# traveller59/spconv

Hardware: NVIDIA H100
Metric: active-voxels/sec fwd+bwd SubMConv3d 3^3 C=64 (higher is better)
Workload: dtype fp16

## Files before the change

spconv_b200/csrc/gemm_tc.cu:

```cuda
#include "gemm.cuh"
#include "wgmma.cuh"
#include <cuda.h>
#include <atomic>
#include <mutex>
#include <stdlib.h>

namespace spx {

constexpr int TC_TILE_M = 128;
constexpr int TC_CONS_WARPS = 8;
constexpr int TC_PROD_WARPS = 2;
constexpr int TC_PROD_THREADS = TC_PROD_WARPS * 32;
constexpr int TC_TMA_WARP = TC_CONS_WARPS + TC_PROD_WARPS;
constexpr int TC_SCHED_WARP = TC_TMA_WARP + 1;
constexpr int TC_THREADS = 3 * 128;
constexpr int TC_INFO_DEPTH = 4;
constexpr int TC_INFO_READERS = TC_PROD_WARPS + TC_CONS_WARPS + 1;
constexpr int TC_MAX_STAGES = 8;
constexpr int TC_SMEM_BUDGET = 200 * 1024;

struct TcParams {
    const uint8_t *x;
    int xb;
    int span_b, b_subtiles, b_sub_bytes, b_bytes, b_mn_major, b_kstep16_mn;
    int b_transposed;
    const float *w;
    int c_in, c_out;
    int w_inner_elems;
    int span_b_elems;
    int n;
    int ab_bf16;
    int stages, a_stage_bytes, stage_bytes, idx_bytes;
    int64_t rows;
    const int32_t *tile_table;
    const int32_t *sched_rec;
    int *sched_state;
    const int32_t *argsort;
    int kv, words, reverse;
    void *y;
    int out_dtype;
    int epi_mode;
    const void *bias;
    int act; float alpha;
    const float *scale, *bias_f32;
    const int8_t *output_add;
    float output_add_scale;
    const float *in_scale, *add_scale, *out_scale;
};

struct BitIter {
    uint32_t m0, m1, m2, m3;
    __device__ __forceinline__ BitIter(const uint32_t (&t)[4]) : m0(t[0]), m1(t[1]), m2(t[2]), m3(t[3]) {}
    __device__ __forceinline__ int next() {
        if (m0) { int b = __ffs(m0) - 1; m0 &= m0 - 1; return b; }
        if (m1) { int b = __ffs(m1) - 1; m1 &= m1 - 1; return 32 + b; }
        if (m2) { int b = __ffs(m2) - 1; m2 &= m2 - 1; return 64 + b; }
        if (m3) { int b = __ffs(m3) - 1; m3 &= m3 - 1; return 96 + b; }
        return -1;
    }
};

template <int OUT>
__device__ __forceinline__ void store2(uint8_t *dst, float a, float b) {
    if constexpr (OUT == SPX_F32) {
        *reinterpret_cast<float2 *>(dst) = make_float2(a, b);
    } else if constexpr (OUT == SPX_F16) {
        *reinterpret_cast<__half2 *>(dst) = __floats2half2_rn(a, b);
    } else if constexpr (OUT == SPX_BF16) {
        *reinterpret_cast<__nv_bfloat162 *>(dst) = __floats2bfloat162_rn(a, b);
    } else {
        const int qa = (int)fminf(fmaxf(rintf(a), -128.f), 127.f), qb = (int)fminf(fmaxf(rintf(b), -128.f), 127.f);
        *reinterpret_cast<uint16_t *>(dst) = (uint16_t)((uint32_t)(uint8_t)(int8_t)qa | ((uint32_t)(uint8_t)(int8_t)qb << 8));
    }
}

template <int OUT> struct OutElem { static constexpr int bytes = OUT == SPX_F32 ? 4 : (OUT == SPX_I8 ? 1 : 2); };

template <int OUT>
__device__ __forceinline__ float load_bias(const void *bias, int j) {
    if constexpr (OUT == SPX_F32) return ((const float *)bias)[j];
    else if constexpr (OUT == SPX_F16) return __half2float(((const __half *)bias)[j]);
    else return __bfloat162float(((const __nv_bfloat16 *)bias)[j]);
}

template <int OUT, bool INT8_MODE, int N, typename Acc, bool PLAIN = false>
__device__ __forceinline__ void epilogue_frag(const TcParams &p, const float *ec, const Acc (&acc)[N / 2], int64_t dst_lo,
                                              int64_t dst_hi, int lane) {
    if constexpr (!INT8_MODE && !PLAIN) {
        if (p.bias == nullptr && p.act == SPX_ACT_NONE) {
            epilogue_frag<OUT, false, N, Acc, true>(p, ec, acc, dst_lo, dst_hi, lane);
            return;
        }
    }
    constexpr int EB = OutElem<OUT>::bytes;
    const bool has_bias = !PLAIN && (INT8_MODE ? (p.bias_f32 != nullptr) : (p.bias != nullptr));
#pragma unroll
    for (int h = 0; h < 2; ++h) {
        const int64_t dst = h ? dst_hi : dst_lo;
        if (dst < 0) continue;
        uint8_t *row_ptr = (uint8_t *)p.y + dst * (int64_t)N * EB;
#pragma unroll
        for (int nb = 0; nb < N / 8; ++nb) {
            const int col = nb * 8 + 2 * (lane & 3);
            float f[2];
#pragma unroll
            for (int j = 0; j < 2; ++j) {
                const Acc v = acc[nb * 4 + 2 * h + j];
                if constexpr (!INT8_MODE) {
                    f[j] = (float)v;
                    if (has_bias) f[j] += ec[col + j];
                } else {
                    f[j] = (float)(int32_t)v * ec[col + j];
                    if (has_bias) f[j] += ec[N + col + j];
                    if (p.output_add) f[j] += (float)p.output_add[dst * (int64_t)N + col + j] * p.output_add_scale;
                }
                if (!PLAIN && p.act != SPX_ACT_NONE) f[j] = apply_act(f[j], p.act, p.alpha);
            }
            store2<OUT>(row_ptr + col * EB, f[0], f[1]);
        }
    }
}

template <int OUT, int N>
__device__ __forceinline__ void epilogue_fp8(const TcParams &p, const float *ec, const float (&acc)[N / 2],
                                             int64_t dst_lo, int64_t dst_hi, int lane, float add_s, float out_s) {
    constexpr int EB = OUT == SPX_F32 ? 4 : (OUT == SPX_E4M3 ? 1 : 2);
    const float *bias = p.bias_f32 ? ec + N : nullptr;
    const void *add = (const void *)p.output_add;
#pragma unroll
    for (int h = 0; h < 2; ++h) {
        const int64_t dst = h ? dst_hi : dst_lo;
        if (dst < 0) continue;
        uint8_t *row_ptr = (uint8_t *)p.y + dst * (int64_t)N * EB;
#pragma unroll
        for (int nb = 0; nb < N / 8; ++nb) {
            const int col = nb * 8 + 2 * (lane & 3);
            float f[2];
#pragma unroll
            for (int j = 0; j < 2; ++j) {
                const float a = add ? load_out_elem<OUT>(add, dst * (int64_t)N + col + j) : 0.f;
                f[j] = fp8_epilogue(acc[nb * 4 + 2 * h + j], ec[col + j], bias, col + j, add != nullptr, a, add_s,
                                    p.act, p.alpha);
            }
            if constexpr (OUT == SPX_E4M3)
                *reinterpret_cast<uint16_t *>(row_ptr + col) = float2_to_e4m3x2(__fdiv_rn(f[0], out_s), __fdiv_rn(f[1], out_s));
            else
                store2<OUT>(row_ptr + col * EB, f[0], f[1]);
        }
    }
}

template <int KIND, int N, typename Acc>
__device__ __forceinline__ void mma_step(Acc (&acc)[N / 2], uint64_t a, uint64_t b, int b_mn, int bf16) {
    if constexpr (KIND == KIND_F16) {
        if (bf16) {
            if (b_mn) Wgmma<N>::template bf16<0, 1>(acc, a, b, 1u);
            else Wgmma<N>::template bf16<0, 0>(acc, a, b, 1u);
        } else {
            if (b_mn) Wgmma<N>::template f16<0, 1>(acc, a, b, 1u);
            else Wgmma<N>::template f16<0, 0>(acc, a, b, 1u);
        }
    } else if constexpr (KIND == KIND_TF32) {
        Wgmma<N>::tf32(acc, a, b, 1u);
    } else if constexpr (KIND == KIND_I8) {
        Wgmma<N>::s8(acc, a, b, 1u);
    } else {
        Wgmma<N>::e4m3(acc, a, b, 1u);
    }
}

template <int KIND, int CPR, int N>
__device__ __forceinline__ void tc_gather_gemm_body(const CUtensorMap &tmap_w, const TcParams &p) {
    using Acc = typename std::conditional<KIND == KIND_I8, int32_t, float>::type;
    constexpr int LG_CPR = CPR == 2 ? 1 : CPR == 4 ? 2 : CPR == 8 ? 3 : CPR == 16 ? 4 : 5;
    constexpr int RPI = 32 / CPR;
    constexpr int XB = CPR * 16;
    constexpr int SPAN_A = XB < 128 ? XB : 128;
    constexpr int LG_SPAN_A = SPAN_A == 128 ? 7 : (SPAN_A == 64 ? 6 : 5);
    constexpr int A_SUB_BYTES = TC_TILE_M * SPAN_A;
    constexpr int A_SUBTILES = XB / SPAN_A;
    constexpr int Q_A = SPAN_A / 32;
    constexpr int ROWS_PW = TC_TILE_M / TC_PROD_WARPS;
    constexpr int ITERS = ROWS_PW / RPI > 0 ? ROWS_PW / RPI : 1;
    static_assert(ROWS_PW * CPR >= 32, "a producer warp must cover at least one full cp.async instruction");

    extern __shared__ __align__(1024) uint8_t smem_raw[];
    const uint32_t raw_addr = smem_u32(smem_raw);
    const uint32_t pad = (1024u - (raw_addr & 1023u)) & 1023u;
    uint8_t *smem = smem_raw + pad;
    const uint32_t smem_base = raw_addr + pad;

    const uint32_t idx_off = (uint32_t)p.stages * p.stage_bytes;
    uint64_t *bars = reinterpret_cast<uint64_t *>(smem + idx_off + 2u * p.idx_bytes);
    uint64_t *full = bars;
    uint64_t *empty = bars + TC_MAX_STAGES;
    uint64_t *idx_full = bars + 2 * TC_MAX_STAGES;
    uint64_t *idx_empty = bars + 2 * TC_MAX_STAGES + 2;
    uint64_t *info_full = bars + 2 * TC_MAX_STAGES + 4;
    uint64_t *info_empty = bars + 2 * TC_MAX_STAGES + 4 + TC_INFO_DEPTH;
    int32_t *info = reinterpret_cast<int32_t *>(bars + 2 * TC_MAX_STAGES + 4 + 2 * TC_INFO_DEPTH);
    float *ec = reinterpret_cast<float *>(smem + idx_off + 2u * p.idx_bytes + 1024u);

    const int warp = threadIdx.x >> 5;
    const int lane = threadIdx.x & 31;
    const int64_t num_tiles = (p.rows + TC_TILE_M - 1) / TC_TILE_M;

    auto read_info = [&](int n, uint32_t (&tm)[4]) -> int {
        const int e = n & (TC_INFO_DEPTH - 1);
        mbar_wait_silent(&info_full[e], (uint32_t)((n / TC_INFO_DEPTH) & 1));
        const volatile int32_t *r = info + e * 8;
        const int tile = r[0];
        tm[0] = (uint32_t)r[1]; tm[1] = (uint32_t)r[2]; tm[2] = (uint32_t)r[3]; tm[3] = (uint32_t)r[4];
        __syncwarp();
        if (lane == 0) mbar_arrive(&info_empty[e]);
        return tile;
    };

    if (threadIdx.x == 0) {
        for (int s = 0; s < p.stages; ++s) {
            mbar_init(&full[s], TC_PROD_THREADS + 1);
            mbar_init(&empty[s], TC_CONS_WARPS);
        }
        for (int a = 0; a < 2; ++a) {
            mbar_init(&idx_full[a], 1);
            mbar_init(&idx_empty[a], TC_PROD_WARPS + TC_CONS_WARPS);
        }
        for (int e = 0; e < TC_INFO_DEPTH; ++e) {
            mbar_init(&info_full[e], 1);
            mbar_init(&info_empty[e], TC_INFO_READERS);
        }
        mbar_fence_init();
        tma_prefetch_desc(&tmap_w);
    }
    for (int j = threadIdx.x; j < N; j += TC_THREADS) {
        if constexpr (KIND == KIND_I8) {
            ec[j] = __ldg(p.scale + j);
            if (p.bias_f32) ec[N + j] = __ldg(p.bias_f32 + j);
        } else if constexpr (KIND == KIND_E4M3) {
            ec[j] = __fmul_rn(__ldg(p.in_scale), __ldg(p.scale + j));
            if (p.bias_f32) ec[N + j] = __ldg(p.bias_f32 + j);
        } else if (p.bias) {
            if constexpr (KIND == KIND_TF32) ec[j] = load_bias<SPX_F32>(p.bias, j);
            else ec[j] = p.out_dtype == SPX_F16 ? load_bias<SPX_F16>(p.bias, j) : load_bias<SPX_BF16>(p.bias, j);
        }
    }
    __syncthreads();

    if (warp >= TC_CONS_WARPS && warp < TC_TMA_WARP) {
        const int pw = warp - TC_CONS_WARPS;
        const int r0 = lane >> LG_CPR;
        const uint32_t byte_in_row = (uint32_t)(lane & (CPR - 1)) << 4;
        const uint8_t *x_lane = p.x + byte_in_row;
        uint32_t dst_off[ITERS];
#pragma unroll
        for (int itc = 0; itc < ITERS; ++itc) {
            const uint32_t row_in_tile = (uint32_t)(pw * ROWS_PW + r0 + itc * RPI);
            const uint32_t sub = byte_in_row >> LG_SPAN_A;
            const uint32_t within = byte_in_row & (uint32_t)(SPAN_A - 1);
            dst_off[itc] = sub * (uint32_t)A_SUB_BYTES + swizzle_offset((row_in_tile << LG_SPAN_A) + within, SPAN_A);
        }
        int stage = 0; uint32_t phase = 0;
        for (int n = 0;; ++n) {
            uint32_t tm[4];
            if (read_info(n, tm) < 0) break;
            const int buf = n & 1;
            mbar_wait_silent(&idx_full[buf], (uint32_t)((n >> 1) & 1));
            const int32_t *idx_lane = reinterpret_cast<const int32_t *>(smem + idx_off + (size_t)buf * p.idx_bytes) +
                                      pw * ROWS_PW + r0;
            BitIter it(tm);
            int k = it.next();
            int32_t ridx[ITERS];
            if (k >= 0) {
#pragma unroll
                for (int itc = 0; itc < ITERS; ++itc) ridx[itc] = idx_lane[k * 128 + itc * RPI];
            }
            while (k >= 0) {
                mbar_wait_silent(&empty[stage], phase ^ 1u);
                const uint32_t a_stage = smem_base + (uint32_t)stage * p.stage_bytes;
#pragma unroll
                for (int itc = 0; itc < ITERS; ++itc)
                    cp_async_16(a_stage + dst_off[itc], x_lane + (int64_t)max(ridx[itc], 0) * XB,
                                ridx[itc] >= 0 ? 16u : 0u);
                cp_async_mbar_arrive_noinc(&full[stage]);
                k = it.next();
                if (k >= 0) {
#pragma unroll
                    for (int itc = 0; itc < ITERS; ++itc) ridx[itc] = idx_lane[k * 128 + itc * RPI];
                }
                if (++stage == p.stages) { stage = 0; phase ^= 1u; }
            }
            __syncwarp();
            if (lane == 0) mbar_arrive(&idx_empty[buf]);
        }
    } else if (warp == TC_TMA_WARP) {
        int stage = 0; uint32_t phase = 0;
        for (int n = 0;; ++n) {
            uint32_t tm[4];
            if (read_info(n, tm) < 0) break;
            BitIter it(tm);
            for (int k = it.next(); k >= 0; k = it.next()) {
                mbar_wait_silent(&empty[stage], phase ^ 1u);
                const int kw = p.reverse ? p.kv - 1 - k : k;
                const uint32_t b_stage = smem_base + (uint32_t)stage * p.stage_bytes + p.a_stage_bytes;
                if (p.b_transposed) {
                    const int i4s = p.c_in >> 2;
                    const float *wk = p.w + (int64_t)kw * p.c_in;
                    for (int q = lane; q < p.c_out * i4s; q += 32) {
                        const int o = q / i4s, i4 = (q - o * i4s) * 4;
                        const float4 v = __ldg(reinterpret_cast<const float4 *>(wk + (int64_t)o * p.kv * p.c_in + i4));
                        const uint32_t kb = (uint32_t)o * 4u;
                        const uint32_t sub = kb / (uint32_t)p.span_b, within = kb % (uint32_t)p.span_b;
                        const float vv[4] = {v.x, v.y, v.z, v.w};
#pragma unroll
                        for (int t = 0; t < 4; ++t) {
                            const uint32_t off = sub * (uint32_t)p.b_sub_bytes +
                                                 swizzle_offset((uint32_t)(i4 + t) * (uint32_t)p.span_b + within, (uint32_t)p.span_b);
                            asm volatile("st.shared.f32 [%0], %1;" ::"r"(b_stage + off), "f"(vv[t]) : "memory");
                        }
                    }
                    fence_proxy_async_smem();
                    __syncwarp();
                    if (lane == 0) mbar_arrive(&full[stage]);
                } else if (lane == 0) {
                    mbar_arrive_expect_tx(&full[stage], (uint32_t)p.b_bytes);
                    for (int sb = 0; sb < p.b_subtiles; ++sb)
                        tma_load_2d(b_stage + sb * p.b_sub_bytes, &tmap_w, &full[stage],
                                    kw * p.w_inner_elems + sb * p.span_b_elems, 0);
                }
                __syncwarp();
                if (++stage == p.stages) { stage = 0; phase ^= 1u; }
            }
        }
    } else if (warp == TC_SCHED_WARP) {
        const uint32_t blk_bytes = (uint32_t)(p.kv + 1) * 512u;
        for (int n = 0;; ++n) {
            const int b = n & 1, e = n & (TC_INFO_DEPTH - 1);
            mbar_wait_silent(&idx_empty[b], (uint32_t)(((n >> 1) & 1) ^ 1));
            mbar_wait_silent(&info_empty[e], (uint32_t)(((n / TC_INFO_DEPTH) & 1) ^ 1));
            int tile = -1;
            if (lane == 0) {
                const int ticket = atomicAdd(p.sched_state, 1);
                int4 r0 = make_int4(-1, 1, 0, 0), r1 = make_int4(0, 0, 0, 0);
                if ((int64_t)ticket < num_tiles) {
                    const int4 *rp = reinterpret_cast<const int4 *>(p.sched_rec + (int64_t)ticket * TT_REC_INTS);
                    r0 = __ldg(rp); r1 = __ldg(rp + 1);
                }
                tile = r0.x;
                int32_t *dst = info + e * 8;
                dst[0] = r0.x; dst[1] = r0.y; dst[2] = r0.z; dst[3] = r0.w; dst[4] = r1.x;
                if (tile >= 0) {
                    mbar_arrive_expect_tx(&idx_full[b], blk_bytes);
                    bulk_copy_g2s(smem_base + idx_off + (uint32_t)b * p.idx_bytes,
                                  p.tile_table + (int64_t)tile * (p.kv + 1) * 128, blk_bytes, &idx_full[b]);
                }
                mbar_arrive(&info_full[e]);
            }
            tile = __shfl_sync(0xffffffffu, tile, 0);
            if (tile < 0) break;
        }
        if (lane == 0) {
            __threadfence();
            const int done = atomicAdd(p.sched_state + 1, 1);
            if (done == (int)gridDim.x - 1) {
                p.sched_state[0] = 0;
                p.sched_state[1] = 0;
                __threadfence();
            }
        }
        __syncwarp();
    } else if (warp < TC_CONS_WARPS) {
        const int wg = warp >> 2;
        int stage = 0; uint32_t phase = 0;
        const uint64_t a_hi = gmma_desc_hi(16u, 8u * SPAN_A, SPAN_A);
        const uint64_t b_hi = p.b_mn_major ? gmma_desc_hi((uint32_t)p.b_sub_bytes, 8u * p.span_b, p.span_b)
                                           : gmma_desc_hi(16u, 8u * p.span_b, p.span_b);
        const uint32_t b_sub16 = (uint32_t)p.b_sub_bytes >> 4;
        Acc acc[N / 2];
        for (int local = 0;; ++local) {
            uint32_t tm[4];
            const int tile = read_info(local, tm);
            if (tile < 0) break;
            int32_t d_lo, d_hi;
            {
                const int buf = local & 1;
                mbar_wait_silent(&idx_full[buf], (uint32_t)((local >> 1) & 1));
                const int32_t *dst = reinterpret_cast<const int32_t *>(smem + idx_off + (size_t)buf * p.idx_bytes) +
                                     p.kv * 128 + wg * 64 + (warp & 3) * 16 + (lane >> 2);
                d_lo = dst[0];
                d_hi = dst[8];
                __syncwarp();
                if (lane == 0) mbar_arrive(&idx_empty[buf]);
            }
#pragma unroll
            for (int i = 0; i < N / 2; ++i) acc[i] = (Acc)0;
            BitIter it(tm);
            int held = -1;
            for (int k = it.next(); k >= 0; k = it.next()) {
                mbar_wait_silent(&full[stage], phase);
                fence_proxy_async_smem();
                const uint32_t a16 = (smem_base + (uint32_t)stage * p.stage_bytes + (uint32_t)(wg * 64 * SPAN_A)) >> 4;
                const uint32_t b16 = (smem_base + (uint32_t)stage * p.stage_bytes + (uint32_t)p.a_stage_bytes) >> 4;
                fence_regs(acc);
                wgmma_fence();
                if (!p.b_mn_major) {
#pragma unroll
                    for (int sub = 0; sub < A_SUBTILES; ++sub) {
                        const uint32_t as = a16 + (uint32_t)sub * (uint32_t)(A_SUB_BYTES >> 4);
                        const uint32_t bs = b16 + (uint32_t)sub * b_sub16;
#pragma unroll
                        for (int jr = 0; jr < Q_A; ++jr)
                            mma_step<KIND, N>(acc, a_hi | (uint64_t)((as + 2u * jr) & 0x3FFFu),
                                              b_hi | (uint64_t)((bs + 2u * jr) & 0x3FFFu), 0, p.ab_bf16);
                    }
                } else {
#pragma unroll
                    for (int sub = 0; sub < A_SUBTILES; ++sub) {
                        const uint32_t as = a16 + (uint32_t)sub * (uint32_t)(A_SUB_BYTES >> 4);
#pragma unroll
                        for (int jr = 0; jr < Q_A; ++jr) {
                            const uint32_t j = (uint32_t)(sub * Q_A + jr);
                            mma_step<KIND, N>(acc, a_hi | (uint64_t)((as + 2u * jr) & 0x3FFFu),
                                              b_hi | (uint64_t)((b16 + j * (uint32_t)p.b_kstep16_mn) & 0x3FFFu), 1,
                                              p.ab_bf16);
                        }
                    }
                }
                wgmma_commit();
                wgmma_wait<1>();
                fence_regs(acc);
                if (held >= 0) {
                    __syncwarp();
                    if (lane == 0) mbar_arrive(&empty[held]);
                }
                held = stage;
                if (++stage == p.stages) { stage = 0; phase ^= 1u; }
            }
            wgmma_wait<0>();
            fence_regs(acc);
            if (held >= 0) {
                __syncwarp();
                if (lane == 0) mbar_arrive(&empty[held]);
            }
            if constexpr (KIND == KIND_F16) {
                if (p.out_dtype == SPX_F16) epilogue_frag<SPX_F16, false, N>(p, ec, acc, d_lo, d_hi, lane);
                else epilogue_frag<SPX_BF16, false, N>(p, ec, acc, d_lo, d_hi, lane);
            } else if constexpr (KIND == KIND_TF32) {
                epilogue_frag<SPX_F32, false, N>(p, ec, acc, d_lo, d_hi, lane);
            } else if constexpr (KIND == KIND_I8) {
                if (p.out_dtype == SPX_I8) epilogue_frag<SPX_I8, true, N>(p, ec, acc, d_lo, d_hi, lane);
                else if (p.out_dtype == SPX_F32) epilogue_frag<SPX_F32, true, N>(p, ec, acc, d_lo, d_hi, lane);
                else epilogue_frag<SPX_F16, true, N>(p, ec, acc, d_lo, d_hi, lane);
            } else {
                const float add_s = p.add_scale ? __ldg(p.add_scale) : 1.f;
                const float out_s = p.out_dtype == SPX_E4M3 ? __ldg(p.out_scale) : 1.f;
                if (p.out_dtype == SPX_E4M3) epilogue_fp8<SPX_E4M3, N>(p, ec, acc, d_lo, d_hi, lane, add_s, out_s);
                else if (p.out_dtype == SPX_F32) epilogue_fp8<SPX_F32, N>(p, ec, acc, d_lo, d_hi, lane, add_s, out_s);
                else if (p.out_dtype == SPX_F16) epilogue_fp8<SPX_F16, N>(p, ec, acc, d_lo, d_hi, lane, add_s, out_s);
                else epilogue_fp8<SPX_BF16, N>(p, ec, acc, d_lo, d_hi, lane, add_s, out_s);
            }
        }
    }

    __syncthreads();
}

template <int KIND, int CPR, int N>
__global__ void __launch_bounds__(TC_THREADS, 1)
tc_gather_gemm_kernel(const __grid_constant__ CUtensorMap tmap_w, const TcParams p) {
    tc_gather_gemm_body<KIND, CPR, N>(tmap_w, p);
}

template <int CPR, int N>
__global__ void __launch_bounds__(TC_THREADS, 1)
tc_gather_gemm_fp8_kernel(const __grid_constant__ CUtensorMap tmap_w, const TcParams p) {
    tc_gather_gemm_body<KIND_E4M3, CPR, N>(tmap_w, p);
}

typedef CUresult (*EncodeTiledFn)(CUtensorMap *, CUtensorMapDataType, cuuint32_t, void *, const cuuint64_t *,
                                  const cuuint64_t *, const cuuint32_t *, const cuuint32_t *, CUtensorMapInterleave,
                                  CUtensorMapSwizzle, CUtensorMapL2promotion, CUtensorMapFloatOOBfill);

static EncodeTiledFn get_encode_fn() {
    static EncodeTiledFn fn = nullptr;
    static std::once_flag once;
    std::call_once(once, [] {
        void *p = nullptr;
        cudaDriverEntryPointQueryResult q;
        if (cudaGetDriverEntryPoint("cuTensorMapEncodeTiled", &p, cudaEnableDefault, &q) == cudaSuccess &&
            q == cudaDriverEntryPointSuccess)
            fn = (EncodeTiledFn)p;
    });
    return fn;
}

int make_weight_tmap(CUtensorMap *tm, const void *w, int dtype, int kv, int c_in, int c_out, int span_bytes) {
    EncodeTiledFn fn = get_encode_fn();
    SPX_REQUIRE(fn != nullptr, "cuTensorMapEncodeTiled entry point not available (driver too old?)");
    const int e = dtype_bytes(dtype);
    CUtensorMapDataType dt = dtype == SPX_F16 ? CU_TENSOR_MAP_DATA_TYPE_FLOAT16
                           : dtype == SPX_BF16 ? CU_TENSOR_MAP_DATA_TYPE_BFLOAT16
                           : dtype == SPX_F32 ? CU_TENSOR_MAP_DATA_TYPE_FLOAT32
                                              : CU_TENSOR_MAP_DATA_TYPE_UINT8;
    cuuint64_t dims[2] = {(cuuint64_t)kv * c_in, (cuuint64_t)c_out};
    cuuint64_t strides[1] = {(cuuint64_t)kv * c_in * e};
    cuuint32_t box[2] = {(cuuint32_t)(span_bytes / e), (cuuint32_t)c_out};
    cuuint32_t estr[2] = {1, 1};
    CUtensorMapSwizzle sw = span_bytes == 128 ? CU_TENSOR_MAP_SWIZZLE_128B
                          : span_bytes == 64 ? CU_TENSOR_MAP_SWIZZLE_64B
                                             : CU_TENSOR_MAP_SWIZZLE_32B;
    CUresult r = fn(tm, dt, 2, const_cast<void *>(w), dims, strides, box, estr, CU_TENSOR_MAP_INTERLEAVE_NONE, sw,
                    CU_TENSOR_MAP_L2_PROMOTION_L2_256B, CU_TENSOR_MAP_FLOAT_OOB_FILL_NONE);
    SPX_REQUIRE(r == CUDA_SUCCESS, "cuTensorMapEncodeTiled failed with %d (kv=%d C=%d K=%d span=%d)", (int)r, kv, c_in,
                c_out, span_bytes);
    return 0;
}

static bool span_ok(int bytes) { return bytes == 32 || bytes == 64 || bytes == 128 || bytes == 256 || bytes == 512; }

static bool tc_shape_ok(int dtype, int kv, int c_in, int c_out, int transpose_w) {
    const int e = dtype_bytes(dtype);
    if (e == 0) return false;
    if (c_in > 256 || c_out > 256) return false;
    if (c_in % 16 || c_out % 16) return false;
    if (!span_ok(c_in * e) || !span_ok(c_out * e)) return false;
    const int cy = transpose_w ? c_in : c_out;
    if (cy % 16 || cy > 256) return false;
    const int xb = (transpose_w ? c_out : c_in) * e;
    if ((dtype == SPX_I8 || dtype == SPX_E4M3) && (c_in % 32 || c_out % 32)) return false;
    size_t stage = align_up((size_t)TC_TILE_M * xb, 1024) + align_up((size_t)c_in * c_out * e, 1024);
    const size_t idx = align_up((size_t)(kv + 1) * 512, 1024);
    if (2 * idx + 2 * stage > (size_t)TC_SMEM_BUDGET) return false;
    return true;
}

static bool tc_operands_aligned(const GatherGemmArgs &a) { return aligned16(a.x) && aligned16(a.w) && aligned16(a.y); }

bool tc_gather_gemm_supported(const GatherGemmArgs &a) {
    if (a.dtype == SPX_I8) return false;
    if (!a.tile_table || !a.tile_mask) return false;
    if (!tc_operands_aligned(a)) return false;
    if (a.dtype == SPX_F32 && a.transpose_w && (runtime_cfg().tf32_dgrad_fma || (a.c_in * 4) % 128)) return false;
    if (((size_t)a.kv * a.c_in * dtype_bytes(a.dtype)) % 16) return false;
    return tc_shape_ok(a.dtype, a.kv, a.c_in, a.c_out, a.transpose_w);
}
bool tc_gather_gemm_int8_supported(const Int8Args &q) {
    if (!q.g.tile_table || !q.g.tile_mask) return false;
    if (!tc_operands_aligned(q.g)) return false;
    if (((size_t)q.g.kv * q.g.c_in) % 16) return false;
    return tc_shape_ok(SPX_I8, q.g.kv, q.g.c_in, q.g.c_out, 0);
}

bool tc_gather_gemm_fp8_supported(const Fp8Args &q) {
    if (!q.g.tile_table || !q.g.tile_mask) return false;
    if (!tc_operands_aligned(q.g)) return false;
    if (((size_t)q.g.kv * q.g.c_in) % 16) return false;
    return tc_shape_ok(SPX_E4M3, q.g.kv, q.g.c_in, q.g.c_out, 0);
}

static int fill_params(const GatherGemmArgs &a, TcParams &p) {
    memset(&p, 0, sizeof(p));
    const int e = dtype_bytes(a.dtype);
    const int cx = a.cx(), cy = a.cy();
    p.x = (const uint8_t *)a.x;
    p.xb = cx * e;
    const int span_a = p.xb < 128 ? p.xb : 128;
    const int wb = a.c_in * e;
    p.b_transposed = (a.dtype == SPX_F32 && a.transpose_w) ? 1 : 0;
    if (p.b_transposed) {
        p.span_b = span_a;
        p.b_subtiles = p.xb / span_a;
        p.b_sub_bytes = cy * span_a;
        p.b_mn_major = 0;
    } else {
        p.span_b = wb < 128 ? wb : 128;
        p.b_subtiles = wb / p.span_b;
        p.b_sub_bytes = a.c_out * p.span_b;
        p.b_mn_major = a.transpose_w;
    }
    p.b_bytes = a.c_out * wb;
    p.b_kstep16_mn = ((32 / e) * p.span_b) >> 4;
    p.w = (const float *)a.w;
    p.c_in = a.c_in; p.c_out = a.c_out;
    p.w_inner_elems = a.c_in;
    p.span_b_elems = p.span_b / e;
    p.n = cy;
    p.ab_bf16 = a.dtype == SPX_BF16;
    p.a_stage_bytes = (int)align_up((size_t)TC_TILE_M * p.xb, 1024);
    p.stage_bytes = p.a_stage_bytes + (int)align_up((size_t)p.b_bytes, 1024);
    p.idx_bytes = (int)align_up((size_t)(a.kv + 1) * 512, 1024);
    p.stages = (TC_SMEM_BUDGET - 2 * p.idx_bytes) / p.stage_bytes;
    if (p.stages > TC_MAX_STAGES) p.stages = TC_MAX_STAGES;
    SPX_REQUIRE(p.stages >= 2, "tc_gather_gemm: tile does not fit shared memory (stage %d bytes)", p.stage_bytes);
    p.rows = a.rows; p.tile_table = a.tile_table; p.argsort = a.argsort;
    {
        const int64_t tiles = div_up64(a.rows, TC_TILE_M);
        p.sched_rec = a.tile_table + tt_blocks_elems(tiles, a.kv);
        static std::atomic<unsigned> next_slot{0};
        const unsigned slot = next_slot.fetch_add(1, std::memory_order_relaxed) % (TT_STATE_INTS / 2);
        p.sched_state = const_cast<int *>(reinterpret_cast<const int *>(p.sched_rec + tiles * TT_REC_INTS)) + 2 * slot;
    }
    p.kv = a.kv; p.words = (a.kv + 31) / 32; p.reverse = a.reverse;
    p.y = a.y; p.out_dtype = a.dtype; p.epi_mode = 0; p.bias = a.bias; p.act = a.act; p.alpha = a.alpha;
    return 0;
}

template <int KIND, int CPR, int N>
static int launch_tc_n(const CUtensorMap &tm, const TcParams &p, cudaStream_t stream) {
    void (*kernel)(const CUtensorMap, const TcParams);
    if constexpr (KIND == KIND_E4M3) kernel = tc_gather_gemm_fp8_kernel<CPR, N>;
    else kernel = tc_gather_gemm_kernel<KIND, CPR, N>;
    const size_t smem = (size_t)p.stages * p.stage_bytes + 2 * (size_t)p.idx_bytes + 1024  + 1024  +
                        2 * N * sizeof(float) ;
    if (!func_configured((const void *)kernel, current_device())) {
        SPX_CHECK_CUDA(cudaFuncSetAttribute(kernel, cudaFuncAttributeMaxDynamicSharedMemorySize,
                                            (int)(TC_SMEM_BUDGET + 2048 + 2 * N * sizeof(float))));
        SPX_CHECK_CUDA(cudaFuncSetAttribute(kernel, cudaFuncAttributePreferredSharedMemoryCarveout, 100));
    }
    const int64_t tiles = div_up64(p.rows, TC_TILE_M);
    const int64_t max_ctas = (int64_t)sm_count();
    const int grid = (int)(tiles < max_ctas ? tiles : max_ctas);
    kernel<<<grid, TC_THREADS, smem, stream>>>(tm, p);
    SPX_CHECK_LAUNCH(KIND == KIND_E4M3 ? "tc_gather_gemm_fp8_kernel" : "tc_gather_gemm_kernel");
    return 0;
}

template <int KIND, int CPR>
static int launch_tc_cpr(const CUtensorMap &tm, const TcParams &p, cudaStream_t stream) {
    switch (p.n) {
        case 16: if constexpr (KIND != KIND_I8 && KIND != KIND_E4M3) return launch_tc_n<KIND, CPR, 16>(tm, p, stream); break;
        case 32: return launch_tc_n<KIND, CPR, 32>(tm, p, stream);
        case 64: return launch_tc_n<KIND, CPR, 64>(tm, p, stream);
        case 128: if constexpr (CPR != 32) return launch_tc_n<KIND, CPR, 128>(tm, p, stream); break;
        case 256: if constexpr (KIND != KIND_TF32 && CPR != 32) return launch_tc_n<KIND, CPR, 256>(tm, p, stream); break;
    }
    set_error("tc_gather_gemm: unsupported output channel count %d", p.n);
    return 2;
}

template <int KIND>
static int launch_tc(const CUtensorMap &tm, const TcParams &p, cudaStream_t stream) {
    switch (p.xb >> 4) {
        case 2: if constexpr (KIND != KIND_TF32) return launch_tc_cpr<KIND, 2>(tm, p, stream); break;
        case 4: return launch_tc_cpr<KIND, 4>(tm, p, stream);
        case 8: return launch_tc_cpr<KIND, 8>(tm, p, stream);
        case 16: return launch_tc_cpr<KIND, 16>(tm, p, stream);
        case 32: if constexpr (KIND != KIND_I8 && KIND != KIND_E4M3) return launch_tc_cpr<KIND, 32>(tm, p, stream); break;
    }
    set_error("tc_gather_gemm: unsupported row bytes %d", p.xb);
    return 2;
}

int tc_gather_gemm(const GatherGemmArgs &a, cudaStream_t stream) {
    TcParams p;
    if (fill_params(a, p)) return 2;
    CUtensorMap tm;
    if (make_weight_tmap(&tm, a.w, a.dtype, a.kv, a.c_in, a.c_out, p.b_transposed ? 128 : p.span_b)) return 2;
    if (a.dtype == SPX_F32) return launch_tc<KIND_TF32>(tm, p, stream);
    return launch_tc<KIND_F16>(tm, p, stream);
}

int tc_gather_gemm_int8(const Int8Args &q, cudaStream_t stream) {
    TcParams p;
    if (fill_params(q.g, p)) return 2;
    p.out_dtype = q.out_dtype;
    p.epi_mode = 1;
    p.scale = q.scale; p.bias_f32 = q.bias_f32; p.output_add = q.output_add;
    p.output_add_scale = q.output_add_scale;
    CUtensorMap tm;
    if (make_weight_tmap(&tm, q.g.w, SPX_I8, q.g.kv, q.g.c_in, q.g.c_out, p.span_b)) return 2;
    return launch_tc<KIND_I8>(tm, p, stream);
}

int tc_gather_gemm_fp8(const Fp8Args &q, cudaStream_t stream) {
    TcParams p;
    if (fill_params(q.g, p)) return 2;
    p.out_dtype = q.out_dtype;
    p.epi_mode = 2;
    p.scale = q.w_scale; p.bias_f32 = q.bias_f32; p.output_add = (const int8_t *)q.output_add;
    p.in_scale = q.in_scale; p.add_scale = q.add_scale; p.out_scale = q.out_scale;
    CUtensorMap tm;
    if (make_weight_tmap(&tm, q.g.w, SPX_E4M3, q.g.kv, q.g.c_in, q.g.c_out, p.span_b)) return 2;
    return launch_tc<KIND_E4M3>(tm, p, stream);
}

}
```

Baseline: 534.0 million.

## Pack two kernel offsets per pipeline stage for small channel counts

When a row holds at most 128 bytes and shared memory allows it, each pipeline stage now carries two kernel-offset slots, each with its own A gather and B weight tile. Producer, TMA and consumer warps walk the offset bitmask two at a time and issue both slots' wgmmas under one commit. This halves the number of mbarrier handshakes and commit/wait rounds per offset for small-C convolutions, where each per-offset GEMM is tiny. The cost is fewer, larger stages, which reduces pipeline depth.

```diff
diff --git a/spconv_b200/csrc/gemm_tc.cu b/spconv_b200/csrc/gemm_tc.cu
--- a/spconv_b200/csrc/gemm_tc.cu
+++ b/spconv_b200/csrc/gemm_tc.cu
@@ -18,6 +18,7 @@
 constexpr int TC_INFO_READERS = TC_PROD_WARPS + TC_CONS_WARPS + 1;
 constexpr int TC_MAX_STAGES = 8;
 constexpr int TC_SMEM_BUDGET = 200 * 1024;
+constexpr bool tc_pair_offsets(int cpr) { return cpr <= 8; }
 
 struct TcParams {
     const uint8_t *x;
@@ -30,7 +31,10 @@
     int span_b_elems;
     int n;
     int ab_bf16;
-    int stages, a_stage_bytes, stage_bytes, idx_bytes;
+    int stages, a_stage_bytes, idx_bytes;
+    int slot_bytes;
+    int pair;
+    int stage_bytes;
     int64_t rows;
     const int32_t *tile_table;
     const int32_t *sched_rec;
@@ -60,6 +64,17 @@
     }
 };
 
+struct StageWalk {
+    BitIter it;
+    bool two;
+    __device__ __forceinline__ StageWalk(const uint32_t (&t)[4], bool two_) : it(t), two(two_) {}
+    __device__ __forceinline__ bool next(int &a, int &b) {
+        a = it.next();
+        b = two && a >= 0 ? it.next() : -1;
+        return a >= 0;
+    }
+};
+
 template <int OUT>
 __device__ __forceinline__ void store2(uint8_t *dst, float a, float b) {
     if constexpr (OUT == SPX_F32) {
@@ -183,6 +198,7 @@
     constexpr int ROWS_PW = TC_TILE_M / TC_PROD_WARPS;
     constexpr int ITERS = ROWS_PW / RPI > 0 ? ROWS_PW / RPI : 1;
     static_assert(ROWS_PW * CPR >= 32, "a producer warp must cover at least one full cp.async instruction");
+    constexpr bool PAIR = tc_pair_offsets(CPR);
 
     extern __shared__ __align__(1024) uint8_t smem_raw[];
     const uint32_t raw_addr = smem_u32(smem_raw);
@@ -267,26 +283,32 @@
             mbar_wait_silent(&idx_full[buf], (uint32_t)((n >> 1) & 1));
             const int32_t *idx_lane = reinterpret_cast<const int32_t *>(smem + idx_off + (size_t)buf * p.idx_bytes) +
                                       pw * ROWS_PW + r0;
-            BitIter it(tm);
-            int k = it.next();
-            int32_t ridx[ITERS];
-            if (k >= 0) {
-#pragma unroll
-                for (int itc = 0; itc < ITERS; ++itc) ridx[itc] = idx_lane[k * 128 + itc * RPI];
-            }
-            while (k >= 0) {
+            auto load_rows = [&](int k, int32_t (&r)[ITERS]) {
+                if (k >= 0) {
+#pragma unroll
+                    for (int itc = 0; itc < ITERS; ++itc) r[itc] = idx_lane[k * 128 + itc * RPI];
+                }
+            };
+            auto gather = [&](uint32_t slot, const int32_t (&r)[ITERS]) {
+#pragma unroll
+                for (int itc = 0; itc < ITERS; ++itc)
+                    cp_async_16(slot + dst_off[itc], x_lane + (int64_t)max(r[itc], 0) * XB, r[itc] >= 0 ? 16u : 0u);
+            };
+            StageWalk walk(tm, PAIR && p.pair);
+            int ka, kb;
+            walk.next(ka, kb);
+            int32_t ra[ITERS], rb[ITERS];
+            load_rows(ka, ra);
+            load_rows(kb, rb);
+            while (ka >= 0) {
                 mbar_wait_silent(&empty[stage], phase ^ 1u);
                 const uint32_t a_stage = smem_base + (uint32_t)stage * p.stage_bytes;
-#pragma unroll
-                for (int itc = 0; itc < ITERS; ++itc)
-                    cp_async_16(a_stage + dst_off[itc], x_lane + (int64_t)max(ridx[itc], 0) * XB,
-                                ridx[itc] >= 0 ? 16u : 0u);
+                gather(a_stage, ra);
+                if (kb >= 0) gather(a_stage + p.slot_bytes, rb);
                 cp_async_mbar_arrive_noinc(&full[stage]);
-                k = it.next();
-                if (k >= 0) {
-#pragma unroll
-                    for (int itc = 0; itc < ITERS; ++itc) ridx[itc] = idx_lane[k * 128 + itc * RPI];
-                }
+                walk.next(ka, kb);
+                load_rows(ka, ra);
+                load_rows(kb, rb);
                 if (++stage == p.stages) { stage = 0; phase ^= 1u; }
             }
             __syncwarp();
@@ -297,35 +319,43 @@
         for (int n = 0;; ++n) {
             uint32_t tm[4];
             if (read_info(n, tm) < 0) break;
-            BitIter it(tm);
-            for (int k = it.next(); k >= 0; k = it.next()) {
+            StageWalk walk(tm, PAIR && p.pair);
+            for (int ka, kb; walk.next(ka, kb);) {
                 mbar_wait_silent(&empty[stage], phase ^ 1u);
-                const int kw = p.reverse ? p.kv - 1 - k : k;
                 const uint32_t b_stage = smem_base + (uint32_t)stage * p.stage_bytes + p.a_stage_bytes;
+                const int nk = kb >= 0 ? 2 : 1;
                 if (p.b_transposed) {
                     const int i4s = p.c_in >> 2;
-                    const float *wk = p.w + (int64_t)kw * p.c_in;
-                    for (int q = lane; q < p.c_out * i4s; q += 32) {
-                        const int o = q / i4s, i4 = (q - o * i4s) * 4;
-                        const float4 v = __ldg(reinterpret_cast<const float4 *>(wk + (int64_t)o * p.kv * p.c_in + i4));
-                        const uint32_t kb = (uint32_t)o * 4u;
-                        const uint32_t sub = kb / (uint32_t)p.span_b, within = kb % (uint32_t)p.span_b;
-                        const float vv[4] = {v.x, v.y, v.z, v.w};
-#pragma unroll
-                        for (int t = 0; t < 4; ++t) {
-                            const uint32_t off = sub * (uint32_t)p.b_sub_bytes +
-                                                 swizzle_offset((uint32_t)(i4 + t) * (uint32_t)p.span_b + within, (uint32_t)p.span_b);
-                            asm volatile("st.shared.f32 [%0], %1;" ::"r"(b_stage + off), "f"(vv[t]) : "memory");
+                    for (int j = 0; j < nk; ++j) {
+                        const int k = j ? kb : ka;
+                        const float *wk = p.w + (int64_t)(p.reverse ? p.kv - 1 - k : k) * p.c_in;
+                        const uint32_t b_slot = b_stage + (uint32_t)j * p.slot_bytes;
+                        for (int q = lane; q < p.c_out * i4s; q += 32) {
+                            const int o = q / i4s, i4 = (q - o * i4s) * 4;
+                            const float4 v = __ldg(reinterpret_cast<const float4 *>(wk + (int64_t)o * p.kv * p.c_in + i4));
+                            const uint32_t ob = (uint32_t)o * 4u;
+                            const uint32_t sub = ob / (uint32_t)p.span_b, within = ob % (uint32_t)p.span_b;
+                            const float vv[4] = {v.x, v.y, v.z, v.w};
+#pragma unroll
+                            for (int t = 0; t < 4; ++t) {
+                                const uint32_t off = sub * (uint32_t)p.b_sub_bytes +
+                                                     swizzle_offset((uint32_t)(i4 + t) * (uint32_t)p.span_b + within, (uint32_t)p.span_b);
+                                asm volatile("st.shared.f32 [%0], %1;" ::"r"(b_slot + off), "f"(vv[t]) : "memory");
+                            }
                         }
                     }
                     fence_proxy_async_smem();
                     __syncwarp();
                     if (lane == 0) mbar_arrive(&full[stage]);
                 } else if (lane == 0) {
-                    mbar_arrive_expect_tx(&full[stage], (uint32_t)p.b_bytes);
-                    for (int sb = 0; sb < p.b_subtiles; ++sb)
-                        tma_load_2d(b_stage + sb * p.b_sub_bytes, &tmap_w, &full[stage],
-                                    kw * p.w_inner_elems + sb * p.span_b_elems, 0);
+                    mbar_arrive_expect_tx(&full[stage], (uint32_t)(nk * p.b_bytes));
+                    for (int j = 0; j < nk; ++j) {
+                        const int k = j ? kb : ka;
+                        const int kw = p.reverse ? p.kv - 1 - k : k;
+                        for (int sb = 0; sb < p.b_subtiles; ++sb)
+                            tma_load_2d(b_stage + (uint32_t)j * p.slot_bytes + sb * p.b_sub_bytes, &tmap_w, &full[stage],
+                                        kw * p.w_inner_elems + sb * p.span_b_elems, 0);
+                    }
                 }
                 __syncwarp();
                 if (++stage == p.stages) { stage = 0; phase ^= 1u; }
@@ -375,6 +405,7 @@
         const uint64_t b_hi = p.b_mn_major ? gmma_desc_hi((uint32_t)p.b_sub_bytes, 8u * p.span_b, p.span_b)
                                            : gmma_desc_hi(16u, 8u * p.span_b, p.span_b);
         const uint32_t b_sub16 = (uint32_t)p.b_sub_bytes >> 4;
+        const uint32_t slot16 = (uint32_t)p.slot_bytes >> 4;
         Acc acc[N / 2];
         for (int local = 0;; ++local) {
             uint32_t tm[4];
@@ -393,39 +424,50 @@
             }
 #pragma unroll
             for (int i = 0; i < N / 2; ++i) acc[i] = (Acc)0;
-            BitIter it(tm);
+            StageWalk walk(tm, PAIR && p.pair);
             int held = -1;
-            for (int k = it.next(); k >= 0; k = it.next()) {
+            for (int ka, kb; walk.next(ka, kb);) {
                 mbar_wait_silent(&full[stage], phase);
                 fence_proxy_async_smem();
                 const uint32_t a16 = (smem_base + (uint32_t)stage * p.stage_bytes + (uint32_t)(wg * 64 * SPAN_A)) >> 4;
                 const uint32_t b16 = (smem_base + (uint32_t)stage * p.stage_bytes + (uint32_t)p.a_stage_bytes) >> 4;
-                fence_regs(acc);
-                wgmma_fence();
-                if (!p.b_mn_major) {
-#pragma unroll
-                    for (int sub = 0; sub < A_SUBTILES; ++sub) {
-                        const uint32_t as = a16 + (uint32_t)sub * (uint32_t)(A_SUB_BYTES >> 4);
-                        const uint32_t bs = b16 + (uint32_t)sub * b_sub16;
-#pragma unroll
-                        for (int jr = 0; jr < Q_A; ++jr)
-                            mma_step<KIND, N>(acc, a_hi | (uint64_t)((as + 2u * jr) & 0x3FFFu),
-                                              b_hi | (uint64_t)((bs + 2u * jr) & 0x3FFFu), 0, p.ab_bf16);
-                    }
-                } else {
-#pragma unroll
-                    for (int sub = 0; sub < A_SUBTILES; ++sub) {
-                        const uint32_t as = a16 + (uint32_t)sub * (uint32_t)(A_SUB_BYTES >> 4);
-#pragma unroll
-                        for (int jr = 0; jr < Q_A; ++jr) {
-                            const uint32_t j = (uint32_t)(sub * Q_A + jr);
-                            mma_step<KIND, N>(acc, a_hi | (uint64_t)((as + 2u * jr) & 0x3FFFu),
-                                              b_hi | (uint64_t)((b16 + j * (uint32_t)p.b_kstep16_mn) & 0x3FFFu), 1,
-                                              p.ab_bf16);
+                auto issue = [&](uint32_t slot) {
+                    const uint32_t a_s = a16 + slot * slot16, b_s = b16 + slot * slot16;
+                    if (!p.b_mn_major) {
+#pragma unroll
+                        for (int sub = 0; sub < A_SUBTILES; ++sub) {
+                            const uint32_t as = a_s + (uint32_t)sub * (uint32_t)(A_SUB_BYTES >> 4);
+                            const uint32_t bs = b_s + (uint32_t)sub * b_sub16;
+#pragma unroll
+                            for (int jr = 0; jr < Q_A; ++jr)
+                                mma_step<KIND, N>(acc, a_hi | (uint64_t)((as + 2u * jr) & 0x3FFFu),
+                                                  b_hi | (uint64_t)((bs + 2u * jr) & 0x3FFFu), 0, p.ab_bf16);
+                        }
+                    } else {
+#pragma unroll
+                        for (int sub = 0; sub < A_SUBTILES; ++sub) {
+                            const uint32_t as = a_s + (uint32_t)sub * (uint32_t)(A_SUB_BYTES >> 4);
+#pragma unroll
+                            for (int jr = 0; jr < Q_A; ++jr) {
+                                const uint32_t j = (uint32_t)(sub * Q_A + jr);
+                                mma_step<KIND, N>(acc, a_hi | (uint64_t)((as + 2u * jr) & 0x3FFFu),
+                                                  b_hi | (uint64_t)((b_s + j * (uint32_t)p.b_kstep16_mn) & 0x3FFFu), 1,
+                                                  p.ab_bf16);
+                            }
                         }
                     }
+                };
+                fence_regs(acc);
+                if (kb >= 0) {
+                    wgmma_fence();
+                    issue(0u);
+                    issue(1u);
+                    wgmma_commit();
+                } else {
+                    wgmma_fence();
+                    issue(0u);
+                    wgmma_commit();
                 }
-                wgmma_commit();
                 wgmma_wait<1>();
                 fence_regs(acc);
                 if (held >= 0) {
@@ -586,8 +628,10 @@
     p.n = cy;
     p.ab_bf16 = a.dtype == SPX_BF16;
     p.a_stage_bytes = (int)align_up((size_t)TC_TILE_M * p.xb, 1024);
-    p.stage_bytes = p.a_stage_bytes + (int)align_up((size_t)p.b_bytes, 1024);
+    p.slot_bytes = p.a_stage_bytes + (int)align_up((size_t)p.b_bytes, 1024);
     p.idx_bytes = (int)align_up((size_t)(a.kv + 1) * 512, 1024);
+    p.pair = tc_pair_offsets(p.xb >> 4) && 2 * p.idx_bytes + 4 * p.slot_bytes <= TC_SMEM_BUDGET;
+    p.stage_bytes = (p.pair + 1) * p.slot_bytes;
     p.stages = (TC_SMEM_BUDGET - 2 * p.idx_bytes) / p.stage_bytes;
     if (p.stages > TC_MAX_STAGES) p.stages = TC_MAX_STAGES;
     SPX_REQUIRE(p.stages >= 2, "tc_gather_gemm: tile does not fit shared memory (stage %d bytes)", p.stage_bytes);
```

Result: no change. 530.2 million, median of 6 (-0.7%).
